# mandt-lab/vbq

Hardware: AMD Instinct MI355X
Metric: quantized latents/sec (32-lambda sweep; one count per (element, lambda) pair and entropy-model build) (higher is better)
Workload: dtype f32; 1 GPU; kodak24_c256 [36864 x 256] f32, 32-lambda sweep, N=10; step = two-pass entropy-model build (quantizer.py:82-150); elements_per_gpu=9437184, lambdas=32, parallelism=element-sharded x1, launch=one HIP graph replay per step

## Files before the change

### include/vbq.h

```cpp
#ifndef VBQ_H_
#define VBQ_H_

#include <stddef.h>
#include <stdint.h>

#ifdef __cplusplus
extern "C" {
#endif

#define VBQ_ABI_VERSION 5

enum {
    VBQ_OK = 0,
    VBQ_ERR_INVALID_ARGUMENT = -1,
    VBQ_ERR_UNSUPPORTED = -2,
    VBQ_ERR_LAUNCH = -3,
    VBQ_ERR_WORKSPACE = -4
};

enum {
    VBQ_LAYOUT_BC = 0,
    VBQ_LAYOUT_CB = 1,
    VBQ_LAYOUT_BC_TO_CB = 2
};
// ... 78 lines not shown

int vbq_histogram_u16(const uint16_t *d_idx, int64_t n_rows, int32_t n_ch, int32_t layout,
                      int32_t n_lambda, int32_t N, int64_t *d_counts, void *stream);

int vbq_histogram_u16_i32(const uint16_t *d_idx, int64_t n_rows, int32_t n_ch, int32_t layout,
                          int32_t n_lambda, int32_t N, int32_t *d_counts, void *stream);

int vbq_histogram_rows_u16(const uint16_t *d_idx, int64_t n_rows, int32_t n_ch, int32_t layout,
                           int32_t n_lambda, int32_t N, void *d_counts, int32_t counts_are_i32,
                           int64_t row_begin, int64_t row_end, void *stream);

int vbq_histogram_models_u16(const uint16_t *d_idx, int64_t n_rows, int32_t n_ch, int32_t n_lambda, int32_t N,
                             void *d_counts, int32_t counts_are_i32, const float *d_lut, int64_t lut_n,
                             float *d_models, void *stream);

int vbq_index_max_u16(const uint16_t *d_idx, int64_t n, uint32_t *d_max, void *stream);

int vbq_moments_f32(const float *d_x, int64_t n_rows, int32_t n_ch, int32_t layout,
                    double *d_out , void *stream);

size_t vbq_numpy_sum_sq_workspace_bytes(int64_t n);
int vbq_numpy_sum_sq_f32(const float *d_x, int64_t n, float *d_out, void *d_workspace, size_t workspace_bytes,
                         void *stream);

size_t vbq_numpy_row_sums_workspace_bytes(int64_t n_rows, int64_t n);
int vbq_numpy_row_sums_f32(const float *d_x, int64_t n_rows, int64_t n, float *d_out, void *d_workspace,
                           size_t workspace_bytes, void *stream);

int vbq_gather_f32(const uint16_t *d_idx, int64_t n_rows, int32_t n_ch, int32_t layout,
                   int32_t n_lambda, int32_t N, const float *d_tab, int32_t tab_per_lambda,
// ... 102 lines not shown
```

### vbq_amd/_lib.py

```python
from __future__ import annotations

import ctypes as C
import os


_LIB = None

c_f32p = C.c_void_p
c_u16p = C.c_void_p

OK = 0
ABI_VERSION = 5
LAYOUT_BC, LAYOUT_CB, LAYOUT_BC_TO_CB = 0, 1, 2
MODE_F32, MODE_F64_SCORE = 0, 1
BMSHJ_PARAMS_PER_CHANNEL = 43
COMM_ID_BYTES = 128

SIGNATURES = {
    "vbq_abi_version": (C.c_int, []),
    "vbq_last_error": (C.c_char_p, []),
    "vbq_solve_grid": (C.c_int, [C.c_int32, C.c_int64, C.c_int32, C.c_int32, C.c_int32, C.POINTER(C.c_int64)]),
    "vbq_device_count": (C.c_int, []),
    "vbq_device_name": (C.c_int, [C.c_int, C.c_char_p, C.c_size_t]),
    "vbq_quantize_workspace_bytes": (C.c_size_t, [C.c_int32, C.c_int32, C.c_int32]),
# ... 15 lines not shown
                                             C.c_void_p, C.c_void_p]),
    "vbq_host_stage_run": (None, [C.c_void_p]),
    "vbq_histogram_rows_u16": (C.c_int, [C.c_void_p, C.c_int64, C.c_int32, C.c_int32, C.c_int32, C.c_int32, C.c_void_p,
                                         C.c_int32, C.c_int64, C.c_int64, C.c_void_p]),
    "vbq_xi_intervals_f64": (C.c_int, [C.c_void_p, C.c_int64, C.c_int32, C.c_void_p, C.c_void_p, C.c_void_p]),
    "vbq_xi_select_f64": (C.c_int, [C.c_void_p, C.c_void_p, C.c_void_p, C.c_int64, C.c_int32, C.c_double, C.c_void_p,
                                    C.c_void_p, C.c_void_p, C.c_void_p, C.c_void_p]),
    "vbq_quantize_notebook_f64": (C.c_int, [C.c_void_p, C.c_void_p, C.c_int64, C.c_void_p, C.POINTER(C.c_double),
                                            C.c_int32, C.c_int32, C.c_void_p, C.c_void_p, C.c_void_p]),
    "vbq_histogram_u16": (C.c_int, [C.c_void_p, C.c_int64, C.c_int32, C.c_int32, C.c_int32, C.c_int32, C.c_void_p,
                                    C.c_void_p]),
    "vbq_histogram_u16_i32": (C.c_int, [C.c_void_p, C.c_int64, C.c_int32, C.c_int32, C.c_int32, C.c_int32,
                                        C.c_void_p, C.c_void_p]),
    "vbq_histogram_models_u16": (C.c_int, [C.c_void_p, C.c_int64, C.c_int32, C.c_int32, C.c_int32, C.c_void_p, C.c_int32,
                                           C.c_void_p, C.c_int64, C.c_void_p, C.c_void_p]),
    "vbq_index_max_u16": (C.c_int, [C.c_void_p, C.c_int64, C.c_void_p, C.c_void_p]),
    "vbq_moments_f32": (C.c_int, [C.c_void_p, C.c_int64, C.c_int32, C.c_int32, C.c_void_p, C.c_void_p]),
    "vbq_numpy_sum_sq_workspace_bytes": (C.c_size_t, [C.c_int64]),
    "vbq_numpy_sum_sq_f32": (C.c_int, [C.c_void_p, C.c_int64, C.c_void_p, C.c_void_p, C.c_size_t, C.c_void_p]),
    "vbq_numpy_row_sums_workspace_bytes": (C.c_size_t, [C.c_int64, C.c_int64]),
    "vbq_numpy_row_sums_f32": (C.c_int, [C.c_void_p, C.c_int64, C.c_int64, C.c_void_p, C.c_void_p, C.c_size_t, C.c_void_p]),
    "vbq_gather_f32": (C.c_int, [C.c_void_p, C.c_int64, C.c_int32, C.c_int32, C.c_int32, C.c_int32, C.c_void_p,
                                 C.c_int32, C.c_void_p, C.c_int32, C.c_void_p]),
    "vbq_rd_sums_u16": (C.c_int, [C.c_void_p, C.c_void_p, C.c_void_p, C.c_int64, C.c_int32, C.c_int32, C.c_int32, C.c_int32,
                                  C.c_void_p, C.c_void_p, C.c_int32, C.c_void_p, C.c_void_p]),
    "vbq_transpose_f32": (C.c_int, [C.c_void_p, C.c_int64, C.c_int64, C.c_void_p, C.c_void_p]),
    "vbq_transpose_planes": (C.c_int, [C.c_void_p, C.c_int64, C.c_int64, C.c_int64, C.c_int32, C.c_void_p, C.c_void_p]),
    "vbq_prep_planes_f32": (C.c_int, [C.c_void_p, C.c_void_p, C.c_int32, C.c_int64, C.c_int32, C.c_void_p, C.c_void_p, C.c_void_p]),
    "vbq_gather_latents_u16": (C.c_int, [C.c_void_p, C.c_int64, C.c_int32, C.c_int32, C.c_int32, C.c_void_p, C.c_void_p,
                                         C.c_void_p, C.c_void_p, C.c_void_p, C.c_void_p, C.c_void_p, C.c_void_p]),
# ... 102 lines not shown
```

### vbq_amd/csrc/vbq_common.h

```cpp
#pragma once

#include <hip/hip_runtime.h>
#include <stdint.h>

#include "vbq.h"

namespace vbq {

void set_error(const char *fmt, ...);

int num_cus();
int fast_debug();
int64_t resident_slots(int per_cu, int reserved);

#define VBQ_REQUIRE(cond, code, ...)            \
    do {                                        \
        if (!(cond)) {                          \
            ::vbq::set_error(__VA_ARGS__);      \
            return (code);                      \
        }                                       \
    } while (0)

#define VBQ_CHECK_LAUNCH(what)                                                        \
    do {                                                                              \
// ... 48 lines not shown
                      float *out_bits, int64_t E, int vec_ok,
                      unsigned long long *level_counts, int wg_per_cu, int reserved, hipStream_t st);

template <int N>
int launch_quant_pruned(const float *mu, const float *sg, int64_t n_per_ch, int64_t ch_stride, int32_t n_ch, const float *table,
                        const Lambdas32 &lam, const float *len, int32_t L, uint16_t *out_idx, int64_t E, int vec_ok, hipStream_t st);

int launch_level_counts_hull10(const float *mu, const float *sg, int64_t n_per_ch, int64_t ch_stride, int32_t n_ch,
                               const float *table, const double *lam, int32_t L, int vec_ok,
                               unsigned long long *level_counts, int reserved, hipStream_t st);

int launch_quant_hull_idx10(const float *mu, const float *sg, int64_t n_per_ch, int64_t ch_stride, int32_t n_ch,
                            const float *table, const double *lam, int32_t L, int vec_ok, uint16_t *out_idx, int64_t E,
                            hipStream_t st);

}
```

### vbq_amd/csrc/vbq_hist.hip

```cpp
#include <stdlib.h>

#include "vbq_common.h"

namespace vbq {
namespace {

#ifndef VBQ_HIST_THREADS
#define VBQ_HIST_THREADS 512
#endif
constexpr int kHistThreads = VBQ_HIST_THREADS;
#ifndef VBQ_HIST_U
#define VBQ_HIST_U 3
#endif

template <int N>
__device__ __forceinline__ unsigned int bin_slot(unsigned int q) { return (q ^ (q >> 6)) & ((2u << N) - 1u); }

__host__ __device__ constexpr int hist_slots(int T) { return T + 1 <= 2048 ? 2048 : (T + 1 <= 4096 ? 4096 : 8192); }
__host__ __device__ constexpr int hist_copies(int T) { return 8192 / hist_slots(T); }

template <int N, int kHistCopies>
__device__ __forceinline__ void hist_add8(unsigned int *h, const uint4 v) {
    unsigned int s[8];
    {
// ... 635 lines not shown
                       int64_t lut_n, float *models, hipStream_t st) {
    const int64_t E = n_rows * (int64_t)n_ch;
    const int vec_ok = reinterpret_cast<uintptr_t>(idx) % 2 == 0;
    if (n_ch <= 65535)
        hipLaunchKernelGGL((k_hist_flat<N, CountT>), dim3(1u, (unsigned)L, (unsigned)n_ch), dim3(kHistThreads), 0, st, idx, (long)n_rows,
                           (long)n_rows, (int)n_ch, (long)E, counts, vec_ok, 2, lut, (long)lut_n, models);
    else
        hipLaunchKernelGGL((k_hist_flat<N, CountT>), dim3(1u, (unsigned)n_ch, (unsigned)L), dim3(kHistThreads), 0, st, idx, (long)n_rows,
                           (long)n_rows, (int)n_ch, (long)E, counts, vec_ok, 1, lut, (long)lut_n, models);
    VBQ_CHECK_LAUNCH("hist_assign");
    return VBQ_OK;
}
}
}

extern "C" int vbq_histogram_models_u16(const uint16_t *d_idx, int64_t n_rows, int32_t n_ch, int32_t n_lambda, int32_t N,
                                        void *d_counts, int32_t counts_are_i32, const float *d_lut, int64_t lut_n,
                                        float *d_models, void *stream) {
    using namespace vbq;
    VBQ_REQUIRE(n_rows >= 0 && n_ch >= 1 && n_lambda >= 1 && n_lambda <= 65535 && n_ch <= 65535, VBQ_ERR_INVALID_ARGUMENT,
                "vbq_histogram_models_u16: bad sizes n_rows=%lld n_ch=%d n_lambda=%d", (long long)n_rows, n_ch, n_lambda);
    VBQ_REQUIRE(d_idx && d_counts && (!d_models || (d_lut && lut_n >= 1)), VBQ_ERR_INVALID_ARGUMENT,
                "vbq_histogram_models_u16: null pointer argument");
    VBQ_REQUIRE(!counts_are_i32 || n_rows <= 0x7fffffffLL, VBQ_ERR_INVALID_ARGUMENT,
                "vbq_histogram_models_u16: %lld rows per channel can overflow 32-bit counters", (long long)n_rows);
    hipStream_t st = reinterpret_cast<hipStream_t>(stream);
    const int64_t n_bins = (int64_t)n_lambda * n_ch * table_size(N);
    const bool fused = (int64_t)n_ch * n_lambda >= 2048 && N >= 4 && N <= 12 && n_rows > 0;
    if (fused) {
#define VBQ_DISPATCH_N(NN)                                                                                                   \
// ... 448 lines not shown
```

### vbq_amd/csrc/vbq_latents.hip

```cpp
#include <atomic>

#include <type_traits>

#include "vbq_common.h"

namespace vbq {
namespace {

__global__ void __launch_bounds__(256)
k_prep_planes(const float *__restrict__ in0, const float *__restrict__ in1, long rows, long cols, float *__restrict__ out0,
              float *__restrict__ out1, int sqrt1, int v4) {
    __shared__ float tile[64][65];
    const bool second = blockIdx.y == 1;
    const float *in = second ? in1 : in0;
    float *out = second ? out1 : out0;
    const int kind = second ? sqrt1 : 0;
    auto f = [kind](float x) { return kind == 0 ? x : sqrtf(kind == 2 ? expf(x) : x); };
    const long ctiles = (cols + 63) / 64;
    const long r0 = ((long)blockIdx.x / ctiles) * 64, c0 = ((long)blockIdx.x % ctiles) * 64;
    if (v4 && r0 + 64 <= rows && c0 + 64 <= cols) {
        float4 v[4];
#pragma unroll
        for (int k = 0; k < 4; ++k) {
            const int i = threadIdx.x + 256 * k, lr = i >> 4, lc = (i & 15) * 4;
// ... 414 lines not shown
    float *sg_cb = reinterpret_cast<float *>(w);
    w += align256(E * sizeof(float));
    uint16_t *idx = reinterpret_cast<uint16_t *>(w);
    w += align256((size_t)n_lambda * E * sizeof(uint16_t));
    const size_t qws = vbq_quantize_workspace_bytes(n_ch, n_lambda, N);
    int rc = vbq_prep_planes_f32(d_means_bc, d_spread_bc, spread_kind, n_rows, n_ch, mu_cb, sg_cb, stream);
    if (rc != VBQ_OK) return rc;
    rc = vbq_quantize_f32(mu_cb, sg_cb, n_rows, n_ch, VBQ_LAYOUT_CB, d_table_lm, d_level_len, h_lambdas, n_lambda, N, VBQ_MODE_F32,
                          idx, nullptr, nullptr, w, qws, stream);
    if (rc != VBQ_OK) return rc;
    return vbq_gather_latents_u16(idx, n_rows, n_ch, n_lambda, N, d_table_sorted, d_level_len, d_models, d_out_zhat, d_out_raw_bits,
                                  d_out_num_bits, nullptr, stream);
}

extern "C" size_t vbq_build_entropy_models_workspace_bytes(int64_t n_rows, int32_t n_ch, int32_t n_lambda, int32_t N) {
    return vbq_compress_latents_workspace_bytes(n_rows, n_ch, n_lambda, N);
}

extern "C" int vbq_build_entropy_models_f32(const float *d_means_bc, const float *d_spread_bc, int32_t spread_kind, int64_t n_rows,
                                            int32_t n_ch, const float *d_table_lm, const double *h_lambdas, int32_t n_lambda,
                                            int32_t N, const float *d_lut_levels, int64_t n_lut_levels, const float *d_lut_ranks,
                                            int64_t n_lut_ranks, int64_t *d_level_counts, float *d_level_len, float *d_raw_models,
                                            void *d_counts, int32_t counts_are_i32, float *d_models, void *d_workspace,
                                            size_t workspace_bytes, int32_t reserved_workgroups, void *stream) {
    using namespace vbq;
    VBQ_REQUIRE(n_rows >= 1 && n_ch >= 1 && n_lambda >= 1 && N >= 0 && N <= 15, VBQ_ERR_INVALID_ARGUMENT,
                "vbq_build_entropy_models_f32: bad sizes");
    VBQ_REQUIRE(d_lut_levels && n_lut_levels > n_rows && d_level_counts && d_level_len && d_raw_models && d_counts,
                VBQ_ERR_INVALID_ARGUMENT, "vbq_build_entropy_models_f32: null pointer argument, or a code-length table shorter than n_rows + 1");
    VBQ_REQUIRE((d_models == nullptr) == (d_lut_ranks == nullptr) && (!d_lut_ranks || n_lut_ranks > n_rows), VBQ_ERR_INVALID_ARGUMENT,
                "vbq_build_entropy_models_f32: d_models and d_lut_ranks go together (n_rows + 1 entries)");
// ... 14 lines not shown
    const size_t qws = vbq_quantize_workspace_bytes(n_ch, n_lambda, N);
    hipStream_t st = reinterpret_cast<hipStream_t>(stream);
    int rc = vbq_prep_planes_f32(d_means_bc, d_spread_bc, spread_kind, n_rows, n_ch, mu_cb, sg_cb, stream);
    if (rc != VBQ_OK) return rc;
    hipError_t e = hipMemsetAsync(d_level_counts, 0, sizeof(int64_t) * (size_t)n_lambda * (size_t)n_ch * (size_t)N1, st);
    if (e != hipSuccess) {
        set_error("vbq_build_entropy_models_f32: hipMemsetAsync: %s", hipGetErrorString(e));
        return VBQ_ERR_LAUNCH;
    }
    rc = vbq_level_counts_f32(mu_cb, sg_cb, n_rows, n_ch, VBQ_LAYOUT_CB, d_table_lm, nullptr, h_lambdas, n_lambda, N, d_level_counts, w, qws,
                              reserved_workgroups, stream);
    if (rc != VBQ_OK) return rc;
    rc = vbq_code_lengths_from_counts(d_level_counts, 0, (int64_t)n_lambda * n_ch * N1, d_lut_levels, n_lut_levels, (int32_t)N1, d_level_len,
                                      d_raw_models, stream);
    if (rc != VBQ_OK) return rc;
    rc = vbq_quantize_rows_f32(mu_cb, sg_cb, n_rows, n_ch, VBQ_LAYOUT_CB, d_table_lm, d_level_len, h_lambdas, n_lambda, N, VBQ_MODE_F32, idx,
                               nullptr, nullptr, w, qws, 0, n_rows, 0, reserved_workgroups, stream);
    if (rc != VBQ_OK) return rc;
    return vbq_histogram_models_u16(idx, n_rows, n_ch, n_lambda, N, d_counts, counts_are_i32, d_lut_ranks, n_lut_ranks, d_models, stream);
}
```

### vbq_amd/csrc/vbq_quantize_fast.hip

```cpp
#include <string.h>

#include "vbq_common.h"

namespace vbq {
namespace {

constexpr int kFastThreads = 256;
#ifndef VBQ_FAST_NE
#define VBQ_FAST_NE 2
#endif
#ifndef VBQ_FAST_WAVES
#define VBQ_FAST_WAVES 4
#endif
#ifndef VBQ_SLOW_INLINE
#define VBQ_SLOW_INLINE __noinline__
#endif
constexpr int kFastNE = VBQ_FAST_NE;

__device__ __forceinline__ float dist_cost(float P, float mu, double rinv) {
    const float d = __fsub_rn(P, mu);
    const float t = (float)__dmul_rn((double)d, rinv);
    const float q = __fmul_rn(t, t);
    return __fmul_rn(0.5f, q);
}
// ... 97 lines not shown
        if (n >= 1) {
            const float cR = __fadd_rn(li.dR, p);
            if (n == 1 || cR < bestR) { bestR = cR; rkR = ((2 * li.posR + 1) << (N - n)) - 1; }
        }
    }
    if (N == 0) return rkL;
    return (bestL <= bestR) ? rkL : rkR;
}

template <int N, int MODE>
__global__ void __launch_bounds__(kFastThreads, VBQ_FAST_WAVES)
k_quant_fast(const float *__restrict__ mu, const float *__restrict__ sg, long n_per_ch, long ch_stride, int C,
             const float *__restrict__ table, Lambdas32 lam, const float *__restrict__ len,
             int L, uint16_t *__restrict__ out_idx, float *__restrict__ out_zhat,
             float *__restrict__ out_bits, long E, int vec_ok, int dbg,
             unsigned long long *__restrict__ level_counts) {
    constexpr int T = table_size(N);
    constexpr int N1 = N + 1;
    constexpr int NE = kFastNE;
    constexpr bool EXTRA = MODE == 1;
    constexpr bool COUNT = MODE == 2;
    const bool never_flag = dbg == 2;
    constexpr int PS = (N1 + 3) & ~3;
    __shared__ float tb[T + 1];
    __shared__ uint32_t scratch[N1 * NE * kFastThreads];
    __shared__ __align__(16) float penl[kMaxLambdaChunk * PS];
    const int c = blockIdx.y;
    if (COUNT) {
        for (int i = threadIdx.x; i < N1 * NE * kFastThreads; i += blockDim.x) scratch[i] = 0;
    }
    for (int i = threadIdx.x; i < T; i += blockDim.x) tb[i] = table[(long)c * T + i];
    int odd = 0;
    for (int i = threadIdx.x; i < L * PS; i += blockDim.x) {
        const int l = i / PS, n = i - l * PS;
        const float p = n < N1 ? __fmul_rn(lam.lam[l], len ? len[((long)l * C + c) * N1 + n] : (float)n) : 0.0f;
        penl[i] = p;
// ... 83 lines not shown
                du[k][n] = vmin(dL, dR);
                g[k] = 2 * g[k] + (below ? 4u : 0u);
                if (COUNT) continue;
                const bool r_better = dR < dL;
                const uint32_t b4 = r_better ? hi4 : lo4;
                const uint32_t better = n < N ? (b4 << (N - n - 1)) + ((1u << (N - n)) - 1u) : (b4 >> 1);
                const uint32_t gap = __float_as_uint(__fsub_rn(dR, dL)) ^ 0x80000000u;
                scratch[(n * NE + k) * kFastThreads + threadIdx.x] = (gap & kWordMask) | better;
            }
        }

        if (resident) {
            set_issue_priority(rot);
            rot += 3u;
        }
        for (int l = 0; l < L; ++l) {
            const float *pp = penl + l * PS;
            float p[N1];
#pragma unroll
            for (int n = 0; n < N1; ++n) p[n] = pp[n];
            uint32_t rank[NE];
            float cst[NE][N1];
            float S[NE];
            uint32_t ne[NE];
#pragma unroll
            for (int n = 0; n < N1; ++n)
#pragma unroll
                for (int k = 0; k < NE; ++k) cst[k][n] = __fadd_rn(du[k][n], p[n]);
#pragma unroll
            for (int k = 0; k < NE; ++k) S[k] = min_of<N1>(cst[k]);
// ... 42 lines not shown
            for (int k = 0; k < NE; ++k) {
                const uint64_t multi = __builtin_amdgcn_uicmp((uint32_t)__popc(ne[k]), (uint32_t)N, 33);
                const uint32_t thr = __float_as_uint(__fmul_rn(S[k], 1.9073486328125e-06f));
                const uint64_t lr_close = __builtin_amdgcn_uicmp(pk[k], thr, 37);
                rank[k] = pk[k] & ((2u << N) - 1u);
                fm[k] = never_flag ? 0ull : (force_slow ? ~0ull : (multi | lr_close));
            }
            uint64_t any_flag = 0;
#pragma unroll
            for (int k = 0; k < NE; ++k) any_flag |= fm[k];
            if (any_flag != 0) {
                const uint32_t lane = __lane_id();
#pragma unroll
                for (int k = 0; k < NE; ++k)
                    if ((fm[k] >> lane) & 1ull) rank[k] = exact_rank_scan<N>(tb, m4[k], s4[k], pp);
            }
            const long o = (long)l * E + base + i0;
            float zh[NE], bt[NE];
            if (EXTRA) {
#pragma unroll
                for (int k = 0; k < NE; ++k) {
                    const uint32_t kk = rank[k] + 1;
                    const int tz = __builtin_ctz(kk);
                    const int lvl = N - tz;
                    const uint32_t pos = kk >> (tz + 1);
                    zh[k] = tb[(1 << lvl) - 1 + pos];
                    bt[k] = len ? len[((long)l * C + c) * N1 + lvl] : (float)lvl;
                }
            }
            if (full) {
// ... 14 lines not shown
                    }
                }
            } else {
#pragma unroll
                for (int k = 0; k < NE; ++k) {
                    if (i0 + k < n_per_ch) {
                        out_idx[o + k] = (uint16_t)rank[k];
                        if (EXTRA) {
                            if (out_zhat) out_zhat[o + k] = zh[k];
                            if (out_bits) out_bits[o + k] = bt[k];
                        }
                    }
                }
            }
        }
    }
    if constexpr (COUNT) {
        __syncthreads();
        for (int i = threadIdx.x; i < L * N1; i += blockDim.x) {
            unsigned int v = 0;
#pragma unroll
            for (int j = 0; j < 16; ++j) {
                const unsigned int w = scratch[i * 16 + j];
                v += (w & 0xffffu) + (w >> 16);
            }
            const int l = i / N1, n = i - l * N1;
            if (v) atomicAdd(&level_counts[((long)l * C + c) * N1 + n], (unsigned long long)v);
        }
    }
}
// ... 865 lines not shown
    const dim3 grid((unsigned)gx, (unsigned)n_ch), block(kFastThreads);
    const int dbg = fast_debug();
    if (level_counts)
        hipLaunchKernelGGL((k_quant_fast<N, 2>), grid, block, 0, st, mu, sg, (long)n_per_ch, (long)ch_stride, (int)n_ch, table,
                           lam, len, (int)L, out_idx, out_zhat, out_bits, (long)E, vec_ok, dbg, level_counts);
    else if (out_zhat || out_bits)
        hipLaunchKernelGGL((k_quant_fast<N, 1>), grid, block, 0, st, mu, sg, (long)n_per_ch, (long)ch_stride, (int)n_ch, table,
                           lam, len, (int)L, out_idx, out_zhat, out_bits, (long)E, vec_ok, dbg, level_counts);
    else
        hipLaunchKernelGGL((k_quant_fast<N, 0>), grid, block, 0, st, mu, sg, (long)n_per_ch, (long)ch_stride, (int)n_ch, table,
                           lam, len, (int)L, out_idx, out_zhat, out_bits, (long)E, vec_ok, dbg, level_counts);
    VBQ_CHECK_LAUNCH("quant_fast");
    return VBQ_OK;
}

template <int N>
int launch_quant_pruned(const float *mu, const float *sg, int64_t n_per_ch, int64_t ch_stride, int32_t n_ch, const float *table,
                        const Lambdas32 &lam, const float *len, int32_t L, uint16_t *out_idx, int64_t E, int vec_ok, hipStream_t st) {
    if (L < 1 || L > kPrunedMaxL) return 1;
    const int64_t npairs = (n_per_ch + 1) / 2;
    int64_t gx = (npairs + 255) / 256;
    int64_t cap = (int64_t)num_cus() * 4 / n_ch;
    if (cap < 1) cap = 1;
    if (gx > cap) gx = cap;
    const int dbg = fast_debug();
    const dim3 grid((unsigned)gx, (unsigned)n_ch), block(256);
#define VBQ_PRUNED_CASE(LLv)                                                                                          \
    case LLv:                                                                                                          \
        hipLaunchKernelGGL((k_quant_pruned<N, LLv>), grid, block, 0, st, mu, sg, (long)n_per_ch, (long)ch_stride, (int)n_ch, \
                           table, lam, len, out_idx, (long)E, vec_ok, dbg);                                            \
// ... 132 lines not shown
                workgroups_per_cu);
    const int reserved = reserved_workgroups < 0 ? 0 : reserved_workgroups;
    if (kernel == VBQ_GRID_K1) {
        int64_t gx = 1;
        bool resident = false;
        quant_fast_grid(n_rows, n_ch, workgroups_per_cu, reserved, false, &gx, &resident);
        h_grid[0] = gx;
        h_grid[2] = resident ? 1 : 0;
    } else {
        h_grid[0] = level_counts_hull_grid(n_rows, n_ch, reserved);
        h_grid[2] = 1;
    }
    h_grid[1] = n_ch;
    return VBQ_OK;
}
```

### vbq_amd/ops.py

```python
from __future__ import annotations

import ctypes as C
from typing import Optional, Sequence

import torch

from . import _lib
from ._lib import LAYOUT_BC, LAYOUT_BC_TO_CB, LAYOUT_CB, MODE_F32, MODE_F64_SCORE, VBQError, check

_LAYOUTS = {"bc": LAYOUT_BC, "cb": LAYOUT_CB, LAYOUT_BC: LAYOUT_BC, LAYOUT_CB: LAYOUT_CB}
_MODES = {"f32": MODE_F32, "f64": MODE_F64_SCORE, MODE_F32: MODE_F32, MODE_F64_SCORE: MODE_F64_SCORE}


def table_size(N: int) -> int:
    return 2 ** (N + 1) - 1


_raw_stream = getattr(torch._C, "_cuda_getCurrentRawStream", None)


def raw_stream(device: torch.device) -> int:
    if _raw_stream is not None:
        return _raw_stream(device.index if device.index is not None else torch.cuda.current_device())
    return torch.cuda.current_stream(device).cuda_stream
# ... 228 lines not shown
    if idx.dim() != 3 or idx.shape[1] != n_ch:
        raise ValueError(f"idx must be planes [L, {n_ch}, rows], got {tuple(idx.shape)}")
    L, _, rows = idx.shape
    T = table_size(N)
    if counts.dtype not in (torch.int64, torch.int32) or tuple(counts.shape) != (L, n_ch, T) or not counts.is_cuda or not counts.is_contiguous():
        raise ValueError(f"counts: expected a contiguous int32 / int64 device tensor of shape {(L, n_ch, T)}")
    if (lut is None) != (models is None):
        raise ValueError("lut and models go together")
    if models is not None:
        lut = _dev(lut, torch.float32, "lut")
        if models.dtype != torch.float32 or tuple(models.shape) != (L, n_ch, T) or not models.is_cuda or not models.is_contiguous():
            raise ValueError(f"models: expected a contiguous f32 device tensor of shape {(L, n_ch, T)}")
    check(_lib.lib().vbq_histogram_models_u16(_ptr(idx), rows, n_ch, L, N, _ptr(counts), int(counts.dtype == torch.int32), _ptr(lut),
                                              lut.numel() if lut is not None else 0, _ptr(models), _stream(idx)),
          "vbq_histogram_models_u16")
    return counts, models


def index_max(idx: torch.Tensor) -> int:
    idx = _dev(idx, torch.uint16, "idx")
    m = torch.zeros(1, dtype=torch.uint32, device=idx.device)
    check(_lib.lib().vbq_index_max_u16(_ptr(idx), idx.numel(), _ptr(m), _stream(idx)), "vbq_index_max_u16")
    return int(m.cpu().item())


def moments(x: torch.Tensor, *, layout="bc", out: Optional[torch.Tensor] = None):
    layout = _LAYOUTS[layout]
    x = _dev(x, torch.float32, "x")
    rows, Cc = _rows_channels(x.shape, layout)
    if out is None:
# ... 282 lines not shown
```

### vbq_amd/pipeline.py

```python
from __future__ import annotations

from typing import Optional, Sequence

import numpy as np
import torch

import ctypes as _C
import glob as _glob
import os as _os

from . import entropy as _entropy
from . import ops
from ._lib import VBQError

_HIP = None


def _hip_runtime():
    global _HIP
    if _HIP is None:
        cands = _glob.glob(_os.path.join(_os.path.dirname(torch.__file__), "lib", "libamdhip64.so*")) + ["libamdhip64.so"]
        for c in cands:
            try:
                _HIP = _C.CDLL(c)
# ... 295 lines not shown
    def _t(self, name, phase):
        if self.timers is not None:
            self.timers(name, phase)

    def lengths(self):
        N1 = self.N + 1
        if self.lut1 is not None:
            ops_out = ops._lib.lib().vbq_code_lengths_from_counts
            ops._lib.check(ops_out(ops._ptr(self.level_counts), 0, self.level_counts.numel(), ops._ptr(self.lut1),
                                   self.lut1.numel(), N1, ops._ptr(self.level_len), ops._ptr(self.raw_models),
                                   ops._stream(self.level_counts)), "vbq_code_lengths_from_counts")
        else:
            self._len_stage.enqueue()
        return self.level_len, self.raw_models

    def pass2(self, mu_cb, sg_cb, level_len):
        if self.world > 1:
            self._slot ^= 1
            self.counts = self._counts2[self._slot]
        self.wait(self._slot)
        main = torch.cuda.current_stream(self.dev)
        self._models_current = False
        if self.side is None and self.world == 1:
            fused = self.lut2 is not None and self.models is not None
            self._t("k1", 0)
            ops.quantize(mu_cb, sg_cb, self.table, self.lambdas, N=self.N, level_len=level_len, layout="cb",
                         out_idx=self.idx, workspace=self.ws, reserved_workgroups=self._reserved())
            self._t("k1", 1)
            self._t("k2", 0)
            ops.histogram_models(self.idx, self.C, self.counts, N=self.N, lut=self.lut2 if fused else None,
                                 models=self.models if fused else None)
            self._t("k2", 1)
            self._models_current = fused
            return self.idx, self.counts
        self.counts.zero_()
        if self.side is None:
            self._t("k1", 0)
            ops.quantize(mu_cb, sg_cb, self.table, self.lambdas, N=self.N, level_len=level_len, layout="cb",
                         out_idx=self.idx, workspace=self.ws, reserved_workgroups=self._reserved())
            self._t("k1", 1)
            self._t("k2", 0)
            ops.histogram(self.idx, self.C, N=self.N, layout="cb", out=self.counts)
            self._t("k2", 1)
        else:
            self.side.wait_stream(main)
            for j, (r0, r1) in enumerate(self.chunks):
# ... 107 lines not shown
```

Baseline: 468.5 billion latents/s.

## Build per-lambda histograms from a delta change stream instead of rescanning indices

The quantize kernel gains an emit mode that records, for each lambda after the first, the elements whose rank differs from the previous lambda, packed as (old<<16|new) entries into per-workgroup segments. A new histogram kernel scans the index plane only for the group's first lambda, then updates the LDS histogram incrementally from the change entries for each later lambda. This avoids re-reading all L index planes in the histogram pass. In exchange the quantizer issues extra ballots, LDS atomics and stores, and needs a change buffer sized by a capacity plan; the path is taken only when the plan marks it as preferred and the lambdas lie in range.

```diff
diff --git a/include/vbq.h b/include/vbq.h
--- a/include/vbq.h
+++ b/include/vbq.h
@@ -116,6 +116,14 @@
                              void *d_counts, int32_t counts_are_i32, const float *d_lut, int64_t lut_n,
                              float *d_models, void *stream);
 
+int vbq_change_stream_plan(int64_t n_rows, int32_t n_ch, int32_t n_lambda, int32_t N, int32_t reserved_workgroups, int64_t *h_plan);
+int vbq_quantize_changes_f32(const float *d_mu_cb, const float *d_sigma_cb, int64_t n_rows, int32_t n_ch, const float *d_table_lm,
+                             const float *d_level_len, const double *h_lambdas, int32_t n_lambda, int32_t N, uint16_t *d_out_idx,
+                             void *d_changes, size_t changes_bytes, int32_t reserved_workgroups, void *stream);
+int vbq_histogram_models_changes_u16(const uint16_t *d_idx, const void *d_changes, size_t changes_bytes, int64_t n_rows,
+                                     int32_t n_ch, int32_t n_lambda, int32_t N, void *d_counts, int32_t counts_are_i32,
+                                     const float *d_lut, int64_t lut_n, float *d_models, int32_t reserved_workgroups, void *stream);
+
 int vbq_index_max_u16(const uint16_t *d_idx, int64_t n, uint32_t *d_max, void *stream);
 
 int vbq_moments_f32(const float *d_x, int64_t n_rows, int32_t n_ch, int32_t layout,
diff --git a/vbq_amd/_lib.py b/vbq_amd/_lib.py
--- a/vbq_amd/_lib.py
+++ b/vbq_amd/_lib.py
@@ -53,6 +53,12 @@
                                         C.c_void_p, C.c_void_p]),
     "vbq_histogram_models_u16": (C.c_int, [C.c_void_p, C.c_int64, C.c_int32, C.c_int32, C.c_int32, C.c_void_p, C.c_int32,
                                            C.c_void_p, C.c_int64, C.c_void_p, C.c_void_p]),
+    "vbq_change_stream_plan": (C.c_int, [C.c_int64, C.c_int32, C.c_int32, C.c_int32, C.c_int32, C.POINTER(C.c_int64)]),
+    "vbq_quantize_changes_f32": (C.c_int, [C.c_void_p, C.c_void_p, C.c_int64, C.c_int32, C.c_void_p, C.c_void_p,
+                                           C.POINTER(C.c_double), C.c_int32, C.c_int32, C.c_void_p, C.c_void_p, C.c_size_t,
+                                           C.c_int32, C.c_void_p]),
+    "vbq_histogram_models_changes_u16": (C.c_int, [C.c_void_p, C.c_void_p, C.c_size_t, C.c_int64, C.c_int32, C.c_int32, C.c_int32,
+                                                   C.c_void_p, C.c_int32, C.c_void_p, C.c_int64, C.c_void_p, C.c_int32, C.c_void_p]),
     "vbq_index_max_u16": (C.c_int, [C.c_void_p, C.c_int64, C.c_void_p, C.c_void_p]),
     "vbq_moments_f32": (C.c_int, [C.c_void_p, C.c_int64, C.c_int32, C.c_int32, C.c_void_p, C.c_void_p]),
     "vbq_numpy_sum_sq_workspace_bytes": (C.c_size_t, [C.c_int64]),
diff --git a/vbq_amd/csrc/vbq_common.h b/vbq_amd/csrc/vbq_common.h
--- a/vbq_amd/csrc/vbq_common.h
+++ b/vbq_amd/csrc/vbq_common.h
@@ -86,4 +86,22 @@
                             const float *table, const double *lam, int32_t L, int vec_ok, uint16_t *out_idx, int64_t E,
                             hipStream_t st);
 
+#ifndef VBQ_CHANGE_GROUPS
+#define VBQ_CHANGE_GROUPS 4
+#endif
+#ifndef VBQ_CHANGE_MIN_LAMBDAS
+#define VBQ_CHANGE_MIN_LAMBDAS 8
+#endif
+constexpr int kChangeGroups = VBQ_CHANGE_GROUPS;
+constexpr int kChangeMinLambdas = VBQ_CHANGE_MIN_LAMBDAS;
+constexpr int kChangeMaxWgs = 64;
+struct ChangeGeom {
+    int64_t gx, cap;
+    int32_t groups;
+    bool resident;
+    bool preferred;
+    size_t counts_bytes, total_bytes;
+};
+bool change_stream_geom(int64_t n_rows, int32_t n_ch, int32_t L, int32_t N, int reserved, ChangeGeom *g);
+
 }
diff --git a/vbq_amd/csrc/vbq_hist.hip b/vbq_amd/csrc/vbq_hist.hip
--- a/vbq_amd/csrc/vbq_hist.hip
+++ b/vbq_amd/csrc/vbq_hist.hip
@@ -673,6 +673,148 @@
 }
 }
 
+namespace vbq {
+namespace {
+constexpr int kChgBatch = 8;
+template <int N, typename CountT>
+__global__ void __launch_bounds__(kHistThreads)
+k_hist_changes(const uint16_t *__restrict__ idx, long n_rows, int C, int L, int groups, const uint32_t *__restrict__ chg_counts,
+               const uint32_t *__restrict__ chg_entries, int gx, long cap, CountT *__restrict__ counts,
+               const float *__restrict__ lut, long lut_n, float *__restrict__ models) {
+    constexpr int T = table_size(N);
+    constexpr int kHistCopies = hist_copies(T);
+    static_assert(kHistCopies == 4 && T + 1 == 2048, "laid out for the 2047 bins of N = 10");
+    __shared__ __align__(16) unsigned int h[8192];
+    extern __shared__ unsigned int fill[];
+    const int c = (int)blockIdx.y, grp = (int)blockIdx.x;
+    const int l0 = (int)((long)grp * L / groups), l1 = (int)((long)(grp + 1) * L / groups);
+    const long E = n_rows * (long)C;
+    const int lane = threadIdx.x & 63;
+    for (int i = threadIdx.x; i < (l1 - l0) * gx; i += kHistThreads) {
+        const unsigned int n = chg_counts[((long)c * L + l0) * gx + i];
+        fill[i] = n < (unsigned long)cap ? n : (unsigned int)cap;
+    }
+#pragma unroll
+    for (int r = 0; r < 2048 / kHistThreads; ++r)
+        reinterpret_cast<uint4 *>(h)[(int)threadIdx.x + r * kHistThreads] = make_uint4(0, 0, 0, 0);
+    __syncthreads();
+    {
+        const uint16_t *src0 = idx + (long)l0 * E + (long)c * n_rows;
+        const long head_max = (long)(((16u - (unsigned)(reinterpret_cast<uintptr_t>(src0) & 15u)) & 15u) >> 1);
+        const long head = head_max < n_rows ? head_max : n_rows;
+        const uint16_t *src = src0 + head;
+        const long n_body = n_rows - head, noct = n_body >> 3;
+        constexpr int U = 3;
+        long q = threadIdx.x;
+        for (; (q - lane) + 63 + (long)(U - 1) * kHistThreads < noct; q += (long)U * kHistThreads) {
+            uint4 A[U];
+#pragma unroll
+            for (int u = 0; u < U; ++u) A[u] = *reinterpret_cast<const uint4 *>(src + (q + (long)u * kHistThreads) * 8);
+#pragma unroll
+            for (int u = 0; u < U; ++u) hist_add8<N, kHistCopies>(h, A[u]);
+        }
+        for (; q < noct; q += kHistThreads) {
+            const uint4 v = *reinterpret_cast<const uint4 *>(src + q * 8);
+            const unsigned int w[4] = {v.x, v.y, v.z, v.w};
+#pragma unroll
+            for (int k = 0; k < 4; ++k) {
+                atomicAdd(&h[kHistCopies * bin_slot<N>(w[k] & 0xffffu)], 1u);
+                atomicAdd(&h[kHistCopies * bin_slot<N>(w[k] >> 16)], 1u);
+            }
+        }
+        for (long i = noct * 8 + threadIdx.x; i < n_body; i += kHistThreads) atomicAdd(&h[kHistCopies * bin_slot<N>(src[i])], 1u);
+        if ((long)threadIdx.x < head) atomicAdd(&h[kHistCopies * bin_slot<N>(src0[threadIdx.x])], 1u);
+    }
+    constexpr int FI = (T + kHistThreads - 1) / kHistThreads;
+    unsigned int *hc = h + (lane & (kHistCopies - 1));
+    for (int l = l0; l < l1; ++l) {
+        if (l > l0) {
+            const unsigned int *fl = fill + (l - l0) * gx;
+            long tot = 0;
+            for (int b = 0; b < gx; ++b) tot += fl[b];
+            const uint32_t *seg0 = chg_entries + ((long)c * (L - 1) + (l - 1)) * gx * cap;
+            for (long i0 = 0; i0 < tot; i0 += (long)kChgBatch * kHistThreads) {
+                uint32_t e[kChgBatch];
+#pragma unroll
+                for (int r = 0; r < kChgBatch; ++r) {
+                    long i = i0 + threadIdx.x + (long)r * kHistThreads;
+                    const bool ok = i < tot;
+                    int b = 0;
+                    while (ok && i >= (long)fl[b]) { i -= fl[b]; ++b; }
+                    e[r] = ok ? __builtin_nontemporal_load(seg0 + (long)b * cap + i) : 0u;
+                }
+#pragma unroll
+                for (int r = 0; r < kChgBatch; ++r) {
+                    const unsigned int nw = bin_slot<N>(e[r] & 0xffffu), od = bin_slot<N>(e[r] >> 16);
+                    if (nw != od) {
+                        atomicAdd(&hc[kHistCopies * nw], 1u);
+                        atomicAdd(&hc[kHistCopies * od], 0xffffffffu);
+                    }
+                }
+            }
+        }
+        __syncthreads();
+        unsigned int v[FI];
+#pragma unroll
+        for (int r = 0; r < FI; ++r) {
+            const int i = (int)threadIdx.x + r * kHistThreads;
+            const int ii = i < T ? i : T - 1;
+            const uint4 q4 = reinterpret_cast<const uint4 *>(h)[bin_slot<N>(ii)];
+            v[r] = (q4.x + q4.y) + (q4.z + q4.w);
+        }
+        __syncthreads();
+        CountT *dst = counts + ((long)l * C + c) * T;
+#pragma unroll
+        for (int r = 0; r < FI; ++r) {
+            const int i = (int)threadIdx.x + r * kHistThreads;
+            if (i < T) dst[i] = (CountT)v[r];
+        }
+        if (models) {
+            float m[FI];
+#pragma unroll
+            for (int r = 0; r < FI; ++r) m[r] = lut[(long)v[r] < lut_n ? (long)v[r] : lut_n - 1];
+            float *mdst = models + ((long)l * C + c) * T;
+#pragma unroll
+            for (int r = 0; r < FI; ++r) {
+                const int i = (int)threadIdx.x + r * kHistThreads;
+                if (i < T) mdst[i] = m[r];
+            }
+        }
+    }
+}
+}
+}
+
+extern "C" int vbq_histogram_models_changes_u16(const uint16_t *d_idx, const void *d_changes, size_t changes_bytes, int64_t n_rows,
+                                                int32_t n_ch, int32_t n_lambda, int32_t N, void *d_counts, int32_t counts_are_i32,
+                                                const float *d_lut, int64_t lut_n, float *d_models, int32_t reserved_workgroups,
+                                                void *stream) {
+    using namespace vbq;
+    VBQ_REQUIRE(d_idx && d_changes && d_counts && (!d_models || (d_lut && lut_n >= 1)), VBQ_ERR_INVALID_ARGUMENT,
+                "vbq_histogram_models_changes_u16: null pointer argument");
+    ChangeGeom g;
+    VBQ_REQUIRE(change_stream_geom(n_rows, n_ch, n_lambda, N, reserved_workgroups < 0 ? 0 : reserved_workgroups, &g),
+                VBQ_ERR_UNSUPPORTED, "vbq_histogram_models_changes_u16: the change-stream route does not apply to n_rows=%lld "
+                "n_ch=%d n_lambda=%d N=%d (vbq_change_stream_plan)", (long long)n_rows, n_ch, n_lambda, N);
+    VBQ_REQUIRE(changes_bytes >= g.total_bytes, VBQ_ERR_WORKSPACE,
+                "vbq_histogram_models_changes_u16: change stream of %zu bytes given, %zu needed", changes_bytes, g.total_bytes);
+    const uint32_t *cc = reinterpret_cast<const uint32_t *>(d_changes);
+    const uint32_t *ce = reinterpret_cast<const uint32_t *>(reinterpret_cast<const char *>(d_changes) + g.counts_bytes);
+    hipStream_t st = reinterpret_cast<hipStream_t>(stream);
+    const dim3 grid((unsigned)g.groups, (unsigned)n_ch), block(kHistThreads);
+    const size_t lds = sizeof(unsigned int) * (size_t)((n_lambda + g.groups - 1) / g.groups) * (size_t)g.gx;
+    if (counts_are_i32)
+        hipLaunchKernelGGL((k_hist_changes<10, unsigned int>), grid, block, lds, st, d_idx, (long)n_rows, (int)n_ch, (int)n_lambda,
+                           (int)g.groups, cc, ce, (int)g.gx, (long)g.cap, reinterpret_cast<unsigned int *>(d_counts), d_lut,
+                           (long)lut_n, d_models);
+    else
+        hipLaunchKernelGGL((k_hist_changes<10, unsigned long long>), grid, block, lds, st, d_idx, (long)n_rows, (int)n_ch,
+                           (int)n_lambda, (int)g.groups, cc, ce, (int)g.gx, (long)g.cap,
+                           reinterpret_cast<unsigned long long *>(d_counts), d_lut, (long)lut_n, d_models);
+    VBQ_CHECK_LAUNCH("hist_changes");
+    return VBQ_OK;
+}
+
 extern "C" int vbq_histogram_models_u16(const uint16_t *d_idx, int64_t n_rows, int32_t n_ch, int32_t n_lambda, int32_t N,
                                         void *d_counts, int32_t counts_are_i32, const float *d_lut, int64_t lut_n,
                                         float *d_models, void *stream) {
diff --git a/vbq_amd/csrc/vbq_latents.hip b/vbq_amd/csrc/vbq_latents.hip
--- a/vbq_amd/csrc/vbq_latents.hip
+++ b/vbq_amd/csrc/vbq_latents.hip
@@ -452,7 +452,10 @@
 }
 
 extern "C" size_t vbq_build_entropy_models_workspace_bytes(int64_t n_rows, int32_t n_ch, int32_t n_lambda, int32_t N) {
-    return vbq_compress_latents_workspace_bytes(n_rows, n_ch, n_lambda, N);
+    size_t need = vbq_compress_latents_workspace_bytes(n_rows, n_ch, n_lambda, N);
+    vbq::ChangeGeom g;
+    if (need && vbq::change_stream_geom(n_rows, n_ch, n_lambda, N, 0, &g) && g.preferred) need += vbq::align256(g.total_bytes);
+    return need;
 }
 
 extern "C" int vbq_build_entropy_models_f32(const float *d_means_bc, const float *d_spread_bc, int32_t spread_kind, int64_t n_rows,
@@ -497,6 +500,21 @@
     rc = vbq_code_lengths_from_counts(d_level_counts, 0, (int64_t)n_lambda * n_ch * N1, d_lut_levels, n_lut_levels, (int32_t)N1, d_level_len,
                                       d_raw_models, stream);
     if (rc != VBQ_OK) return rc;
+    {
+        ChangeGeom g;
+        char *chg = w + align256(qws);
+        bool ok = change_stream_geom(n_rows, n_ch, n_lambda, N, reserved_workgroups < 0 ? 0 : reserved_workgroups, &g) &&
+                  g.preferred &&
+                  (size_t)(chg - static_cast<char *>(d_workspace)) + g.total_bytes <= workspace_bytes;
+        for (int i = 0; ok && i < n_lambda; ++i) ok = h_lambdas[i] >= 1.9e-12 && h_lambdas[i] <= 1.8e19;
+        if (ok) {
+            rc = vbq_quantize_changes_f32(mu_cb, sg_cb, n_rows, n_ch, d_table_lm, d_level_len, h_lambdas, n_lambda, N, idx, chg,
+                                          g.total_bytes, reserved_workgroups, stream);
+            if (rc != VBQ_OK) return rc;
+            return vbq_histogram_models_changes_u16(idx, chg, g.total_bytes, n_rows, n_ch, n_lambda, N, d_counts, counts_are_i32,
+                                                    d_lut_ranks, n_lut_ranks, d_models, reserved_workgroups, stream);
+        }
+    }
     rc = vbq_quantize_rows_f32(mu_cb, sg_cb, n_rows, n_ch, VBQ_LAYOUT_CB, d_table_lm, d_level_len, h_lambdas, n_lambda, N, VBQ_MODE_F32, idx,
                                nullptr, nullptr, w, qws, 0, n_rows, 0, reserved_workgroups, stream);
     if (rc != VBQ_OK) return rc;
diff --git a/vbq_amd/csrc/vbq_quantize_fast.hip b/vbq_amd/csrc/vbq_quantize_fast.hip
--- a/vbq_amd/csrc/vbq_quantize_fast.hip
+++ b/vbq_amd/csrc/vbq_quantize_fast.hip
@@ -135,12 +135,18 @@
              const float *__restrict__ table, Lambdas32 lam, const float *__restrict__ len,
              int L, uint16_t *__restrict__ out_idx, float *__restrict__ out_zhat,
              float *__restrict__ out_bits, long E, int vec_ok, int dbg,
-             unsigned long long *__restrict__ level_counts) {
+             unsigned long long *__restrict__ level_counts, uint32_t *__restrict__ chg_entries = nullptr,
+             uint32_t *__restrict__ chg_counts = nullptr, long chg_cap = 0) {
     constexpr int T = table_size(N);
     constexpr int N1 = N + 1;
     constexpr int NE = kFastNE;
     constexpr bool EXTRA = MODE == 1;
     constexpr bool COUNT = MODE == 2;
+    constexpr bool EMIT = MODE == 3;
+    __shared__ uint32_t chg_fill[EMIT ? kMaxLambdaChunk : 1];
+    if constexpr (EMIT) {
+        if (threadIdx.x < kMaxLambdaChunk) chg_fill[threadIdx.x] = 0;
+    }
     const bool never_flag = dbg == 2;
     constexpr int PS = (N1 + 3) & ~3;
     __shared__ float tb[T + 1];
@@ -254,6 +260,9 @@
             set_issue_priority(rot);
             rot += 3u;
         }
+        uint32_t prev[NE];
+#pragma unroll
+        for (int k = 0; k < NE; ++k) prev[k] = 0;
         for (int l = 0; l < L; ++l) {
             const float *pp = penl + l * PS;
             float p[N1];
@@ -326,6 +335,35 @@
 #pragma unroll
                 for (int k = 0; k < NE; ++k)
                     if ((fm[k] >> lane) & 1ull) rank[k] = exact_rank_scan<N>(tb, m4[k], s4[k], pp);
+            }
+            if constexpr (EMIT) {
+                if (l > 0) {
+                    uint64_t cm[NE], any_change = 0;
+                    uint32_t total = 0;
+#pragma unroll
+                    for (int k = 0; k < NE; ++k) {
+                        cm[k] = __ballot(rank[k] != prev[k] && i0 + k < n_per_ch);
+                        any_change |= cm[k];
+                        total += (uint32_t)__popcll(cm[k]);
+                    }
+                    if (any_change != 0) {
+                        const int leader = __ffsll((long long)any_change) - 1;
+                        uint32_t got = 0;
+                        if ((int)__lane_id() == leader) got = atomicAdd(&chg_fill[l], total);
+                        uint32_t at = __builtin_amdgcn_readlane(got, leader);
+                        uint32_t *seg = chg_entries + (((long)c * (L - 1) + (l - 1)) * gridDim.x + blockIdx.x) * chg_cap;
+#pragma unroll
+                        for (int k = 0; k < NE; ++k) {
+                            const uint32_t slot = __builtin_amdgcn_mbcnt_hi((uint32_t)(cm[k] >> 32),
+                                                                           __builtin_amdgcn_mbcnt_lo((uint32_t)cm[k], at));
+                            if (rank[k] != prev[k] && i0 + k < n_per_ch)
+                                __builtin_nontemporal_store((prev[k] << 16) | rank[k], seg + slot);
+                            at += (uint32_t)__popcll(cm[k]);
+                        }
+                    }
+                }
+#pragma unroll
+                for (int k = 0; k < NE; ++k) prev[k] = rank[k];
             }
             const long o = (long)l * E + base + i0;
             float zh[NE], bt[NE];
@@ -370,6 +408,10 @@
                 }
             }
         }
+    }
+    if constexpr (EMIT) {
+        __syncthreads();
+        if ((int)threadIdx.x < L) chg_counts[((long)c * L + threadIdx.x) * gridDim.x + blockIdx.x] = chg_fill[threadIdx.x];
     }
     if constexpr (COUNT) {
         __syncthreads();
@@ -1265,6 +1307,39 @@
     return VBQ_OK;
 }
 
+bool change_stream_geom(int64_t n_rows, int32_t n_ch, int32_t L, int32_t N, int reserved, ChangeGeom *g) {
+    ChangeGeom z = {};
+    *g = z;
+    if (N != 10 || L < 1 || L > kMaxLambdaChunk || n_rows < 1 || n_ch < 1 || n_ch > 65535 || n_rows > 0x7fffffffLL / 4) return false;
+    int64_t gx = 1;
+    bool resident = false;
+    quant_fast_grid(n_rows, n_ch, 0, reserved, false, &gx, &resident);
+    if (gx > kChangeMaxWgs) return false;
+    g->groups = kChangeGroups < L ? kChangeGroups : L;
+    const int64_t nquads = (n_rows + kFastNE - 1) / kFastNE;
+    const int64_t iters = (nquads + kFastThreads - 1) / kFastThreads;
+    g->gx = gx;
+    g->resident = resident;
+    g->cap = ((iters + gx - 1) / gx) * kFastThreads * kFastNE;
+    g->counts_bytes = (((size_t)n_ch * L * gx * sizeof(uint32_t)) + 255) & ~(size_t)255;
+    g->total_bytes = g->counts_bytes + (size_t)n_ch * (L - 1) * gx * g->cap * sizeof(uint32_t);
+    g->preferred = L >= kChangeMinLambdas && resident && gx <= 8 && (int64_t)n_ch * g->groups >= num_cus();
+    return true;
+}
+
+int launch_quant_fast_changes10(const float *mu, const float *sg, int64_t n_rows, int32_t n_ch, const float *table,
+                                const Lambdas32 &lam, const float *len, int32_t L, uint16_t *out_idx, int vec_ok,
+                                const ChangeGeom &g, void *stream_buf, hipStream_t st) {
+    uint32_t *counts = reinterpret_cast<uint32_t *>(stream_buf);
+    uint32_t *entries = reinterpret_cast<uint32_t *>(reinterpret_cast<char *>(stream_buf) + g.counts_bytes);
+    hipLaunchKernelGGL((k_quant_fast<10, 3>), dim3((unsigned)g.gx, (unsigned)n_ch), dim3(kFastThreads), 0, st, mu, sg, (long)n_rows,
+                       (long)n_rows, (int)n_ch, table, lam, len, (int)L, out_idx, (float *)nullptr, (float *)nullptr,
+                       (long)(n_rows * (int64_t)n_ch), vec_ok | (g.resident ? 4 : 0), fast_debug(), (unsigned long long *)nullptr, entries, counts,
+                       (long)g.cap);
+    VBQ_CHECK_LAUNCH("quant_fast_changes");
+    return VBQ_OK;
+}
+
 template <int N>
 int launch_quant_pruned(const float *mu, const float *sg, int64_t n_per_ch, int64_t ch_stride, int32_t n_ch, const float *table,
                         const Lambdas32 &lam, const float *len, int32_t L, uint16_t *out_idx, int64_t E, int vec_ok, hipStream_t st) {
@@ -1427,3 +1502,42 @@
     h_grid[1] = n_ch;
     return VBQ_OK;
 }
+
+extern "C" int vbq_change_stream_plan(int64_t n_rows, int32_t n_ch, int32_t n_lambda, int32_t N, int32_t reserved_workgroups,
+                                      int64_t *h_plan) {
+    using namespace vbq;
+    VBQ_REQUIRE(h_plan, VBQ_ERR_INVALID_ARGUMENT, "vbq_change_stream_plan: null pointer argument");
+    ChangeGeom g;
+    const bool ok = change_stream_geom(n_rows, n_ch, n_lambda, N, reserved_workgroups < 0 ? 0 : reserved_workgroups, &g);
+    h_plan[0] = ok && g.preferred ? 1 : 0;
+    h_plan[1] = (int64_t)g.total_bytes;
+    h_plan[2] = g.gx;
+    h_plan[3] = g.cap;
+    h_plan[4] = g.groups;
+    h_plan[5] = ok ? 1 : 0;
+    return VBQ_OK;
+}
+
+extern "C" int vbq_quantize_changes_f32(const float *d_mu_cb, const float *d_sigma_cb, int64_t n_rows, int32_t n_ch,
+                                        const float *d_table_lm, const float *d_level_len, const double *h_lambdas,
+                                        int32_t n_lambda, int32_t N, uint16_t *d_out_idx, void *d_changes, size_t changes_bytes,
+                                        int32_t reserved_workgroups, void *stream) {
+    using namespace vbq;
+    VBQ_REQUIRE(d_mu_cb && d_sigma_cb && d_table_lm && h_lambdas && d_out_idx && d_changes, VBQ_ERR_INVALID_ARGUMENT,
+                "vbq_quantize_changes_f32: null pointer argument");
+    ChangeGeom g;
+    VBQ_REQUIRE(change_stream_geom(n_rows, n_ch, n_lambda, N, reserved_workgroups < 0 ? 0 : reserved_workgroups, &g),
+                VBQ_ERR_UNSUPPORTED, "vbq_quantize_changes_f32: the change-stream route does not apply to n_rows=%lld n_ch=%d "
+                "n_lambda=%d N=%d (vbq_change_stream_plan)", (long long)n_rows, n_ch, n_lambda, N);
+    VBQ_REQUIRE(changes_bytes >= g.total_bytes, VBQ_ERR_WORKSPACE, "vbq_quantize_changes_f32: change stream of %zu bytes given, %zu needed",
+                changes_bytes, g.total_bytes);
+    Lambdas32 l32;
+    for (int i = 0; i < kMaxLambdaChunk; ++i) l32.lam[i] = i < n_lambda ? (float)h_lambdas[i] : 0.0f;
+    for (int i = 0; i < n_lambda; ++i)
+        VBQ_REQUIRE(h_lambdas[i] >= 1.9e-12 && h_lambdas[i] <= 1.8e19, VBQ_ERR_UNSUPPORTED,
+                    "vbq_quantize_changes_f32: lambda %g outside the fast kernel's range [1.9e-12, 1.8e19]", h_lambdas[i]);
+    const int vec2_ok = ((reinterpret_cast<uintptr_t>(d_mu_cb) | reinterpret_cast<uintptr_t>(d_sigma_cb)) % 4 == 0) &&
+                        (reinterpret_cast<uintptr_t>(d_out_idx) % 2 == 0);
+    return launch_quant_fast_changes10(d_mu_cb, d_sigma_cb, n_rows, n_ch, d_table_lm, l32, d_level_len, n_lambda, d_out_idx, vec2_ok,
+                                       g, d_changes, reinterpret_cast<hipStream_t>(stream));
+}
diff --git a/vbq_amd/ops.py b/vbq_amd/ops.py
--- a/vbq_amd/ops.py
+++ b/vbq_amd/ops.py
@@ -266,6 +266,73 @@
     check(_lib.lib().vbq_histogram_models_u16(_ptr(idx), rows, n_ch, L, N, _ptr(counts), int(counts.dtype == torch.int32), _ptr(lut),
                                               lut.numel() if lut is not None else 0, _ptr(models), _stream(idx)),
           "vbq_histogram_models_u16")
+    return counts, models
+
+
+def change_stream_plan(rows: int, n_ch: int, L: int, *, N: int = 10, reserved_workgroups: Optional[int] = None) -> dict:
+    p = (C.c_int64 * 6)()
+    check(_lib.lib().vbq_change_stream_plan(rows, n_ch, L, N, -1 if reserved_workgroups is None else int(reserved_workgroups), p),
+          "vbq_change_stream_plan")
+    return {"ok": bool(p[0]), "bytes": int(p[1]), "workgroups_per_channel": int(p[2]), "segment_entries": int(p[3]),
+            "lambda_runs": int(p[4]), "served": bool(p[5])}
+
+
+def quantize_changes(mu_cb: torch.Tensor, sigma_cb: torch.Tensor, table_lm: torch.Tensor, lambdas: Sequence[float], *,
+                     N: int = 10, level_len: Optional[torch.Tensor] = None, out_idx: Optional[torch.Tensor] = None,
+                     changes: Optional[torch.Tensor] = None, reserved_workgroups: Optional[int] = None):
+    mu_cb = _dev(mu_cb, torch.float32, "mu")
+    sigma_cb = _dev(sigma_cb, torch.float32, "sigma")
+    if mu_cb.dim() != 2 or mu_cb.shape != sigma_cb.shape:
+        raise ValueError(f"expected two [C, rows] tensors, got {tuple(mu_cb.shape)} / {tuple(sigma_cb.shape)}")
+    Cc, rows = mu_cb.shape
+    L = len(lambdas)
+    table_lm = _dev(table_lm, torch.float32, "table_lm")
+    if table_lm.numel() != Cc * table_size(N):
+        raise ValueError(f"table_lm has {table_lm.numel()} entries, expected C*T = {Cc}*{table_size(N)}")
+    if level_len is not None:
+        level_len = _dev(level_len, torch.float32, "level_len")
+        if tuple(level_len.shape) != (L, Cc, N + 1):
+            raise ValueError(f"level_len shape {tuple(level_len.shape)} != {(L, Cc, N + 1)}")
+    plan = change_stream_plan(rows, Cc, L, N=N, reserved_workgroups=reserved_workgroups)
+    if not plan["served"]:
+        raise VBQError(f"the change-stream kernels do not serve rows={rows} C={Cc} L={L} N={N}")
+    if out_idx is None:
+        out_idx = torch.empty((L, Cc, rows), dtype=torch.uint16, device=mu_cb.device)
+    elif tuple(out_idx.shape) != (L, Cc, rows) or out_idx.dtype != torch.uint16 or not out_idx.is_cuda or not out_idx.is_contiguous():
+        raise ValueError(f"out_idx: expected a contiguous uint16 device tensor of shape {(L, Cc, rows)}")
+    if changes is None:
+        changes = torch.empty(plan["bytes"], dtype=torch.uint8, device=mu_cb.device)
+    elif changes.dtype != torch.uint8 or changes.numel() < plan["bytes"] or not changes.is_cuda or not changes.is_contiguous():
+        raise ValueError(f"changes: expected a contiguous uint8 device tensor of at least {plan['bytes']} bytes")
+    check(_lib.lib().vbq_quantize_changes_f32(_ptr(mu_cb), _ptr(sigma_cb), rows, Cc, _ptr(table_lm), _ptr(level_len), _doubles(lambdas),
+                                              L, N, _ptr(out_idx), _ptr(changes), changes.numel(),
+                                              -1 if reserved_workgroups is None else int(reserved_workgroups), _stream(mu_cb)),
+          "vbq_quantize_changes_f32")
+    return out_idx, changes
+
+
+def histogram_models_changes(idx: torch.Tensor, changes: torch.Tensor, n_ch: int, counts: torch.Tensor, *, N: int = 10,
+                             lut: Optional[torch.Tensor] = None, models: Optional[torch.Tensor] = None,
+                             reserved_workgroups: Optional[int] = None):
+    idx = _dev(idx, torch.uint16, "idx")
+    if idx.dim() != 3 or idx.shape[1] != n_ch:
+        raise ValueError(f"idx must be planes [L, {n_ch}, rows], got {tuple(idx.shape)}")
+    L, _, rows = idx.shape
+    T = table_size(N)
+    if counts.dtype not in (torch.int64, torch.int32) or tuple(counts.shape) != (L, n_ch, T) or not counts.is_cuda or not counts.is_contiguous():
+        raise ValueError(f"counts: expected a contiguous int32 / int64 device tensor of shape {(L, n_ch, T)}")
+    if (lut is None) != (models is None):
+        raise ValueError("lut and models go together")
+    if models is not None:
+        lut = _dev(lut, torch.float32, "lut")
+        if models.dtype != torch.float32 or tuple(models.shape) != (L, n_ch, T) or not models.is_cuda or not models.is_contiguous():
+            raise ValueError(f"models: expected a contiguous f32 device tensor of shape {(L, n_ch, T)}")
+    if changes.dtype != torch.uint8 or not changes.is_cuda or not changes.is_contiguous():
+        raise ValueError("changes: expected the contiguous uint8 device buffer quantize_changes filled")
+    check(_lib.lib().vbq_histogram_models_changes_u16(_ptr(idx), _ptr(changes), changes.numel(), rows, n_ch, L, N, _ptr(counts),
+                                                      int(counts.dtype == torch.int32), _ptr(lut), lut.numel() if lut is not None else 0,
+                                                      _ptr(models), -1 if reserved_workgroups is None else int(reserved_workgroups),
+                                                      _stream(idx)), "vbq_histogram_models_changes_u16")
     return counts, models
 
 
diff --git a/vbq_amd/pipeline.py b/vbq_amd/pipeline.py
--- a/vbq_amd/pipeline.py
+++ b/vbq_amd/pipeline.py
@@ -333,6 +333,15 @@
             self._len_stage.enqueue()
         return self.level_len, self.raw_models
 
+    def _change_stream(self):
+        if self.world != 1 or self.side is not None or any(not (1.9e-12 <= float(v) <= 1.8e19) for v in self.lambdas):
+            return None
+        plan = ops.change_stream_plan(self.rows, self.C, self.L, N=self.N, reserved_workgroups=self._reserved())
+        if not plan["ok"]:
+            return None
+        return self._kept(("changes", self.L, self.C, self.rows, plan["bytes"], str(self.dev)),
+                          lambda: torch.empty(plan["bytes"], dtype=torch.uint8, device=self.dev))
+
     def pass2(self, mu_cb, sg_cb, level_len):
         if self.world > 1:
             self._slot ^= 1
@@ -342,13 +351,22 @@
         self._models_current = False
         if self.side is None and self.world == 1:
             fused = self.lut2 is not None and self.models is not None
+            changes = self._change_stream()
             self._t("k1", 0)
-            ops.quantize(mu_cb, sg_cb, self.table, self.lambdas, N=self.N, level_len=level_len, layout="cb",
-                         out_idx=self.idx, workspace=self.ws, reserved_workgroups=self._reserved())
+            if changes is not None:
+                ops.quantize_changes(mu_cb, sg_cb, self.table, self.lambdas, N=self.N, level_len=level_len, out_idx=self.idx,
+                                     changes=changes, reserved_workgroups=self._reserved())
+            else:
+                ops.quantize(mu_cb, sg_cb, self.table, self.lambdas, N=self.N, level_len=level_len, layout="cb",
+                             out_idx=self.idx, workspace=self.ws, reserved_workgroups=self._reserved())
             self._t("k1", 1)
             self._t("k2", 0)
-            ops.histogram_models(self.idx, self.C, self.counts, N=self.N, lut=self.lut2 if fused else None,
-                                 models=self.models if fused else None)
+            if changes is not None:
+                ops.histogram_models_changes(self.idx, changes, self.C, self.counts, N=self.N, lut=self.lut2 if fused else None,
+                                             models=self.models if fused else None, reserved_workgroups=self._reserved())
+            else:
+                ops.histogram_models(self.idx, self.C, self.counts, N=self.N, lut=self.lut2 if fused else None,
+                                     models=self.models if fused else None)
             self._t("k2", 1)
             self._models_current = fused
             return self.idx, self.counts
```

Measured after the change: 416.8 billion latents/s. 11.0% lower.
